# thetengda/OKVIS2-X

Measured on AMD Instinct MI355X. Metric: Gauss-Newton iters/sec on 50-KF/2000-landmark window; ATE vs CPU ref, higher is better.
Workload: dtype f64; 1 GPU; 2048 independent S50 windows (50 KF / 2000 landmarks / 16000 reprojections, 49 IMU factors), DENSE_SCHUR + DOGLEG, all tolerances 0; windows_total=2048, windows_per_gpu=2048, parallelism=replicas x1 (one window batch per GPU, no collective in the loop)

## Files before the change

include/okvisgpu.h:

```cpp
#ifndef OKVISGPU_H_
#define OKVISGPU_H_

#include <stdint.h>

#ifdef __cplusplus
extern "C" {
#endif

#define OKVISGPU_ABI_VERSION 6

typedef enum okvisgpu_status {
  OKVISGPU_OK = 0,
  OKVISGPU_ERR_INVALID_ARGUMENT = 1,
  OKVISGPU_ERR_UNSUPPORTED = 2,
  OKVISGPU_ERR_DEVICE = 3,
  OKVISGPU_ERR_OUT_OF_MEMORY = 4,
  OKVISGPU_ERR_NO_PROBLEM = 5,
  OKVISGPU_ERR_NUMERICAL = 6
} okvisgpu_status;

typedef enum okvisgpu_distortion {
  OKVISGPU_DIST_NONE = 0,
  OKVISGPU_DIST_RADTAN = 1,
  OKVISGPU_DIST_EQUIDISTANT = 2,
// ... 225 lines not shown
  const double* sample_gyr_acc;
} okvisgpu_imu_append_batch;
int okvisgpu_imu_append(okvisgpu_ctx* ctx, const okvisgpu_imu_append_batch* batch, int32_t* steps);

typedef struct okvisgpu_graph okvisgpu_graph;
int okvisgpu_graph_load(const char* path, const okvisgpu_camera* cameras, int32_t n_cameras,
                        const okvisgpu_imu_params* imu, okvisgpu_graph** out);
const okvisgpu_problem* okvisgpu_graph_problem(okvisgpu_graph* g);
int okvisgpu_graph_ids(const okvisgpu_graph* g, uint64_t* state_ids, int64_t* state_t_ns, uint64_t* landmark_ids);
void okvisgpu_graph_destroy(okvisgpu_graph* g);
int okvisgpu_graph_save(const okvisgpu_problem* p, const int64_t* state_t_ns, const char* path);

typedef struct okvisgpu_problem_stats {
  int32_t n_windows;
  int32_t cholesky_launches;
  int64_t n_poses, n_speed_biases, n_landmarks, n_landmarks_free, n_extrinsics_free;
  int64_t n_observations, n_visits, n_imu, n_imu_samples, n_pose_priors, n_sb_priors, n_relpose;
  int64_t reduced_dim;
  int64_t s_tiles_nonzero;
  int64_t s_tiles_dense;
  int64_t n_block_pairs, n_visit_segments, n_partial_blocks;
  int64_t arena_bytes;
  int64_t cholesky_split_windows;
} okvisgpu_problem_stats;
int okvisgpu_get_stats(okvisgpu_ctx* ctx, okvisgpu_problem_stats* stats);

int okvisgpu_plan_window(const okvisgpu_problem* problem, int32_t nested_dissection, int64_t* info,
                         uint8_t* tile_nz, int32_t* step_launch, int32_t* natural);

int okvisgpu_get_params(okvisgpu_ctx* ctx);

int okvisgpu_evaluate(okvisgpu_ctx* ctx, int32_t window, double* cost);

int okvisgpu_linearize_reduce(okvisgpu_ctx* ctx, int32_t window, int32_t jacobi_scaling, double mu,
                              double* S, double* rhs, double* cost, int32_t* dim_out);

int okvisgpu_eval_reprojection(okvisgpu_ctx* ctx, int32_t window, double* r, double* J_pose,
                               double* J_landmark);
int okvisgpu_eval_imu(okvisgpu_ctx* ctx, int32_t window, int32_t redo_always, double* r, double* J);
int okvisgpu_eval_relpose(okvisgpu_ctx* ctx, int32_t window, double* r, double* J);
int okvisgpu_eval_host(okvisgpu_ctx* ctx, int32_t window, double* r, double* J);

typedef struct okvisgpu_synth_config {
  int32_t n_keyframes;
  int32_t n_landmarks;
  int32_t n_observations;
// ... 31 lines not shown
```

okvis2-x_amd/csrc/chol_tiles.hpp:

```cpp
#pragma once
#include "dev_clock.hpp"
#include "device_problem.hpp"
#include "okvisgpu_math.hpp"

namespace okg {

constexpr int kLd = kTile + 1;


typedef double dbl4 __attribute__((ext_vector_type(4)));

__device__ __forceinline__ bool cholSelect(const DevProblem& P, int w) {
  const WinState& s = P.st[w];
  return !s.done && s.need_gn && !s.gn_failed;
}

__device__ __forceinline__ int tileBlocks(const DevProblem& P, int w, int k) {
  const int fdim = P.win_fdim[w], g0 = P.win_sgap[2 * w], gl = P.win_sgap[2 * w + 1];
  int end = min(fdim - kTile * k, kTile);
  if (gl > 0 && g0 >= kTile * k && g0 < kTile * (k + 1)) end = min(end, g0 - kTile * k);
  return max(1, (end + 15) >> 4);
}

struct TileSrc {
// ... 297 lines not shown
__host__ __device__ constexpr bool persistentCaller(int kCaller) { return kCaller >= 10; }
template <int kCaller>
__device__ __forceinline__ void xStoreRows16(const double* sX, double* Li, int q, int g, int lane) {
  double2 v[3];
#pragma unroll
  for (int it = 0; it < 3; ++it) {
    const int e = min(64 * g + lane + 192 * it, 511), r = 16 * q + (e >> 5), c = 2 * (e & 31);
    v[it] = double2{(c <= r) ? sX[r * kLd + c] : 0.0, (c + 1 <= r) ? sX[r * kLd + c + 1] : 0.0};
  }
#pragma unroll
  for (int it = 0; it < 3; ++it) {
    const int e = 64 * g + lane + 192 * it, r = 16 * q + (e >> 5), c = 2 * (e & 31);
    if (e < 512 && (!persistentCaller(kCaller) || c <= r)) *gmemw(reinterpret_cast<double2*>(Li + r * kTile + c)) = v[it];
  }
}

__host__ __device__ constexpr bool teamCaller(int kCaller) { return kCaller >= 20; }
constexpr int kPotrfBarriers = 3;
template <int kCaller>
__device__ __forceinline__ void potrfSync(int* sFl, int& tgen, int lane) {
  if (teamCaller(kCaller)) waveBarrier<true>(&sFl[4], tgen, 4, lane);
  else ldsBarrier();
}
template <int kCaller>
__device__ __forceinline__ bool potrfTileBody(const double* Sg, int64_t ld, double* Li, double* workk, double* sA, double* sX,
                                              double* sy, double* sRl, int* sFl, int t, bool haveTile, int tgen0, int nq) {
  const int wave = t >> 6, lane = t & 63;
  int tgen = tgen0;
  CLK_INIT
  if (!haveTile) loadTile(Sg, ld, 0, 0, sA, t);
  nq = __builtin_amdgcn_readfirstlane(nq);
#pragma unroll
  for (int u = 0; u < 16; ++u) {
    const int e = t + 256 * u;
    sX[(e >> 6) * kLd + (e & 63)] = 0.0;
  }
  if (t < 4) sFl[t] = 0;
  potrfSync<kCaller>(sFl, tgen, lane);
  CLK(4)
  if (wave == 0) {
    const int i = lane;
    if (i >= 16 * nq) {
      sX[i * kLd + i] = 1.0;
      sy[kTile + i] = sy[i];
    }
    double xp[8];
#pragma unroll
    for (int k = 0; k < 8; ++k) xp[k] = 0.0;
#pragma unroll 1
    for (int s = 0; s < 2 * nq; ++s) {
      const int c0 = 8 * s;
      CLK(25)
      if (s >= 2 && !waitFlag<true>(&sFl[1], s - 1, &sFl[2])) break;
      CLK(21)
      double r[8], x[8], rl[8];
#pragma unroll
      for (int k = 0; k < 8; ++k) r[k] = sA[i * kLd + c0 + k];
      if (s >= 1) {
#pragma unroll
        for (int hb = 0; hb < 2; ++hb) {
          double Lq[4][8];
#pragma unroll
          for (int c = 0; c < 4; ++c)
// ... 44 lines not shown
      if (s & 1) {
        const int q = s >> 1;
        if (g == 0) xDiag16(sA, sX, q, lane);
        waveBarrier<true>(&sFl[3], gen, 3, lane);
        if (g < q) xOffDiag16(sA, sX, q, g, lane);
        waveBarrier<true>(&sFl[3], gen, 3, lane);
        if (g == 0) yBlock16(sX, sy, q, lane);
        for (int qs = q, qe = q + 1 < nq ? q + 1 : 4; qs < qe; ++qs) xStoreRows16<kCaller>(sX, Li, qs, g, lane);
      }
    }
  }
  potrfSync<kCaller>(sFl, tgen, lane);
  CLK(5)
  if (sFl[2]) return false;
  if (t < kTile) {
    const double y = sy[kTile + t];
    sy[t] = y;
    if (!persistentCaller(kCaller)) gmemw(workk)[t] = y;
  }
  potrfSync<kCaller>(sFl, tgen, lane);
  CLK(10)
  return true;
}
template <int kCaller>
__device__ __noinline__ bool potrfTile(const double* Sg, int64_t ld, double* Li, double* workk, double* sA, double* sX, double* sy,
                                      double* sRl, int* sFl, int t, bool haveTile, int tgen0 = 0, int nq = 4) {
  return potrfTileBody<kCaller>(Sg, ld, Li, workk, sA, sX, sy, sRl, sFl, t, haveTile, tgen0, nq);
}

__device__ __forceinline__ void accToLds(double* s, const dbl4 acc[2][2], int t) {
  const int wave = t >> 6, lane = t & 63;
  const int r0 = 32 * (wave >> 1), c0 = 32 * (wave & 1);
#pragma unroll
  for (int a = 0; a < 2; ++a)
#pragma unroll
    for (int b = 0; b < 2; ++b)
#pragma unroll
      for (int reg = 0; reg < 4; ++reg) s[(r0 + 16 * a + (lane >> 4) + 4 * reg) * kLd + c0 + 16 * b + (lane & 15)] = acc[a][b][reg];
}
__device__ __forceinline__ void accSubToLds(double* s, const dbl4 c[2][2], const dbl4 acc[2][2], int t) {
  const int wave = t >> 6, lane = t & 63;
  const int r0 = 32 * (wave >> 1), c0 = 32 * (wave & 1);
#pragma unroll
  for (int a = 0; a < 2; ++a)
#pragma unroll
    for (int b = 0; b < 2; ++b)
#pragma unroll
      for (int reg = 0; reg < 4; ++reg)
        s[(r0 + 16 * a + (lane >> 4) + 4 * reg) * kLd + c0 + 16 * b + (lane & 15)] = c[a][b][reg] - acc[a][b][reg];
}
// ... 82 lines not shown
__device__ __forceinline__ void panelRhsVector(const double* sX, const double* sy, double* sz, double* sP, int t,
                                               Sync sync = Sync()) {
  const int c = t & 63, q = t >> 6;
  double a = 0.0;
#pragma unroll
  for (int r = 16 * q; r < 16 * q + 16; ++r) a += (r >= c) ? sX[r * kLd + c] * sy[r] : 0.0;
  sP[q * kTile + c] = a;
  sync();
  if (t < kTile) sz[t] = (sP[t] + sP[kTile + t]) + (sP[2 * kTile + t] + sP[3 * kTile + t]);
  sync();
}

__device__ __forceinline__ double panelRhsRow(const double* sA, const double* sz, int t) {
  const int row = t >> 2, q = t & 3;
  double a = 0.0;
#pragma unroll
  for (int c = 16 * q; c < 16 * q + 16; ++c) a += sA[row * kLd + c] * sz[c];
  a += __shfl_xor(a, 1, 64);
  a += __shfl_xor(a, 2, 64);
  return a;
}

template <class Sync = WgSync>
__device__ __forceinline__ void panelTile(const double* Aik, double* Lik, int64_t ld, double* worki, double* sA, const double* sX, const double* sz,
                          int t, double* defer = nullptr, Sync sync = Sync()) {
  loadTile(Aik, ld, 0, 0, sA, t);
  sync();
  dbl4 acc[4];
  mfmaPanelRows(sA, sX, acc, t);
  {
    const int row = t >> 2, q = t & 3;
    const double a = panelRhsRow(sA, sz, t);
    if (q == 0) {
      if (defer) defer[row] = a;
      else worki[row] -= a;
    }
  }
  sync();
  storePanelRows(Lik, ld, acc, t);
}


constexpr int kBsThreads = 1024;
constexpr int kBsPre = 3;
struct BsOps {
  double2 v[kBsPre][2];
  double2 li[2];
};
template <bool UPPER>
__device__ __forceinline__ const double* bsTile(const double* S, int64_t ld, int I, int i) {
  return UPPER ? S + (int64_t)I * kTile * ld + i * kTile : S + (int64_t)i * kTile * ld + I * kTile;
}
template <bool UPPER>
__device__ __forceinline__ void bsLoad(const double* S, int64_t ld, const double* Linv, const int* lst, int I, int vt,
                                       BsOps& o) {
  const int c2 = 2 * (vt & 31), rg = vt >> 5;
#ifdef OKG_BS_DUMMY_DIAG
  const int dummy = I;
#else
  const int dummy = lst[0] > 0 ? lst[1] : I;
#endif
#pragma unroll
// ... 116 lines not shown
```

okvis2-x_amd/csrc/device_problem.hpp:

```cpp
#pragma once

#include <cstdint>

namespace okg {

constexpr int kCamDoubles = 13;
constexpr int kTile = 64;
constexpr int16_t kNoUpdate = 32767;
constexpr int kImuLin = 15 + 15 * 30;
constexpr int kImuState = 526;
constexpr int kHostIn = 40;
constexpr int kHostOut = 1 + kImuLin;

constexpr int kObsLin = 8;
constexpr int kSegHG = 28;
constexpr int kSegUz = 8;
constexpr int kLmGroupVisits = 256;
__host__ __device__ constexpr bool fewWindows(int nWin, int cuCount) { return 4 * nWin <= cuCount; }
constexpr int kLmGroupMax = 64;
constexpr int kLmPartStage = 2048;
constexpr int kAsmLightMax = 24;
constexpr int kManyWindows = 64;
constexpr int kLmgInfo = 8;
constexpr int kImuHess = 465 + 30;
constexpr int kGrpRed = 8;
constexpr int kVisitZ = 18;

enum ContribType : int32_t {
  C_VISIT = 0,
  C_PAIR = 1,
  C_IMU = 2,
// ... 188 lines not shown
  int32_t n_asm_ppl;
  const int32_t* pair_win;
  const int32_t* pair_fi;
  const int32_t* pair_fj;
  const int32_t* pair_cbegin;
  const int32_t* pair_runs;
  const Contrib* pair_contrib;

  double* S;
  double* W;
  double* Linv;
  const int64_t* win_linvoff;
  const int32_t* tile_items;
  const int32_t* chol_root_items;
  int32_t n_chol_roots;
  int32_t n_chol_launches;
  const int32_t* chol_upd_items;
  const int32_t* chol_upd_begin;
  const int32_t* h_upd_begin;
  int32_t chol_schedule;
  const uint8_t* tile_nz;
  const int16_t* tile_fu;
  const int64_t* win_tnzoff;
  int32_t n_tiles;
  double* chol_defer;
  const int64_t* win_defoff;
  double* fwdF;
  const int64_t* win_fwdoff;
  double* sF;   double* sL;
  double* diagF; double* diagL;
  double* hdF;
  double* gF;   double* gL;
  double* rhsF;
  double* yF;   double* yL;
  double* gnF;  double* gnL;
  double* dgF;  double* dgL;
  double* vF;   double* vL;
  double* stepF; double* stepL;

  WinState* st;
  DevOptions opt;
};

constexpr int kTwoPoseOut = 6 + 36 + 7 + 36 + 6;
struct TwoPoseDev {
  int32_t n_edges, n_cam;
// ... 17 lines not shown
```

okvis2-x_amd/csrc/kernels_chol.hip:

```cpp
#include "chol_tiles.hpp"
#include "launch.hpp"

namespace okg {

#ifndef OKG_CHOL_OCC
#define OKG_CHOL_OCC 2
#endif

template <int MODE>
__global__ __launch_bounds__(256, OKG_CHOL_OCC) void k_cholesky(const DevProblem* __restrict__ Pp) {
  const DevProblem& P = *Pp;
  const int w = MODE == 1 ? (int)(blockIdx.x >> 1) : (int)blockIdx.x, part = MODE == 1 ? (int)(blockIdx.x & 1) : 0;
  if (!cholSelect(P, w)) return;
  const int64_t ld = P.win_fpad[w];
  const int T = (int)(ld / kTile);
  const int tL = MODE == 0 ? 0 : P.win_bsplit[2 * w], tS = MODE == 0 ? 0 : P.win_bsplit[2 * w + 1];
  const bool split = MODE != 0 && tS > 0;
  if ((MODE == 1 && part == 1 && !split) || (MODE == 2 && !split)) return;
  const int k0 = !split ? 0 : (MODE == 2 ? tS : (part == 0 ? 0 : tL));
  const int k1 = !split ? T : (MODE == 2 ? T : (part == 0 ? tL : tS));
  const int jEnd = split && MODE == 1 && part == 1 ? tS : T;
  const bool finish = !split || MODE == 2;
  const TileSrc cur = tileSrc(P, w, ld);
  double* W = P.W + P.win_soff[w];
  double* Linv = P.Linv + P.win_linvoff[w];
  const uint8_t* nz = P.tile_nz + P.win_tnzoff[w];
  double* work = P.fwdF + P.win_fwdoff[w];
  double* defer = split ? P.chol_defer + P.win_defoff[w] : nullptr;
  __shared__ double sA[kTile * kLd];
// ... 53 lines not shown
          }
        } else {
          dbl4 c[2][2], acc[2][2];
          loadC(cur.at(i, j, k), ld, c, t);
          mfmaTileNT(aBuf, bBuf, acc, t);
          storeTileSub(Cij, ld, c, acc, t);
        }
        ldsBarrier();
      }
    }
    return inLds;
  };
  if (MODE == 2) {
    for (int k = tL; k < tS; ++k) {
      for (int i = tS; i < T; ++i)
        if (nz[i * T + k] && t < kTile)
          sxDyn[i * kTile + t] -= defer[((size_t)(i - tS) * (tS - tL) + (k - tL)) * kTile + t];
      __syncthreads();
      bandUpdate(k, tS, false);
      __syncthreads();
    }
  }
  bool haveDiag = false;
  for (int k = k0; k < k1; ++k) {
    CLK(11)
    if (t < kTile) sy[t] = sxDyn[k * kTile + t];
    __syncthreads();
    if (!potrfTile<10 + MODE>(cur.at(k, k, k), ld, Linv + (int64_t)k * kTile * kTile, nullptr, sA, sX,
                   sy, sRl, sFl, t, haveDiag, 0, tileBlocks(P, w, k))) {
      if (t == 0) P.st[w].gn_failed = 1;
      return;
    }
    if (t < kTile) sxDyn[k * kTile + t] = sy[t];
    CLK(0)
    tStep = t;
    asm volatile("" : "+v"(tStep));
    panelRhsVector(sX, sy, sy + kTile, sA, t);
    for (int i = k + 1; i < T; ++i)
      if (nz[i * T + k])
        panelTile(cur.at(i, k, k), W + i * kTile * ld + k * kTile, ld, sxDyn + i * kTile, sA, sX, sy + kTile, tStep,
                  i >= jEnd ? defer + ((size_t)(i - tS) * (tS - tL) + (k - tL)) * kTile : nullptr);
    __syncthreads();
    CLK(1)
    haveDiag = bandUpdate(k, 0, true);
  }
  CLK(2)
// ... 223 lines not shown
```

okvis2-x_amd/csrc/runtime.cpp:

```cpp
#include <hip/hip_runtime.h>

#include <algorithm>
#include <array>
#include <cfloat>
#include <chrono>
#include <climits>
#include <cmath>
#include <condition_variable>
#include <cstdio>
#include <cstdlib>
#include <cstring>
#include <functional>
#include <map>
#include <memory>
#include <mutex>
#include <numeric>
#include <stdexcept>
#include <string>
#include <thread>
#include <vector>

#include "../../include/okvisgpu.h"
#include "device_problem.hpp"
#include "launch.hpp"
// ... 91 lines not shown
  std::vector<int32_t> fb_win, fb_kind, fb_index, fb_off, fb_cbegin;
  std::vector<int32_t> win_sgap, f_nat, win_fnat, win_bsplit;
  std::vector<int64_t> win_defoff;
  int64_t defer_total = 0;
  bool any_split = false;
  bool nd = false;
  int lmg_visits = kLmGroupVisits, lmg_lms = kLmGroupMax;
  std::vector<int32_t> chol_root_items;
  int n_chol_launches = 1;
  std::vector<Contrib> fb_contrib;
  std::vector<int32_t> pair_win, pair_fi, pair_fj, pair_cbegin, pair_runs;
  std::vector<int32_t> asm_pp_items, asm_sb_items, asm_ppl_items;
  std::vector<int32_t> chol_upd_items, chol_upd_begin, tile_items;
  int64_t n_panels = 0;
  int64_t n_band_updates = 0;
  int64_t n_band_updates_diag = 0;
  std::vector<Contrib> pair_contrib;
  int64_t s_total = 0, linv_total = 0, fwd_total = 0;
  std::vector<std::vector<uint8_t>> tileNz;
  std::vector<uint8_t> tile_nz;
  std::vector<std::vector<int16_t>> tileFu;
  std::vector<int16_t> tile_fu;
  std::vector<int64_t> win_tnzoff;
  std::vector<int> tileT;
  int f_total = 0;
  int max_fpad = 0;
  int max_panels = 0;
};

template <class T>
void appendN(std::vector<T>& v, const T* src, size_t n) {
  if (n) v.insert(v.end(), src, src + n);
}

bool lossValid(const okvisgpu_loss& L) {
  switch (L.kind) {
    case OKVISGPU_LOSS_NONE: return true;
    case OKVISGPU_LOSS_TOLERANT: return L.a >= 0.0 && L.b > 0.0 && std::isfinite(L.a) && std::isfinite(L.b);
    case OKVISGPU_LOSS_CAUCHY: case OKVISGPU_LOSS_TUKEY: case OKVISGPU_LOSS_HUBER: case OKVISGPU_LOSS_SOFTLONE:
    case OKVISGPU_LOSS_ARCTAN: return L.a > 0.0 && std::isfinite(L.a);
  }
  return false;
}

void lossRho(const okvisgpu_loss& L, double s, double* rho) {
  const double a = L.a;
// ... 168 lines not shown
    }
  }
}

#ifdef OKG_ANALYSE_TIMING
double g_atime[16];
std::chrono::steady_clock::time_point g_alast;
#define ATIME(i)                                                                                    \
  {                                                                                                 \
    const auto now = std::chrono::steady_clock::now();                                             \
    g_atime[i] += std::chrono::duration<double, std::milli>(now - g_alast).count();                 \
    g_alast = now;                                                                                  \
  }
#else
#define ATIME(i)
#endif

void symbolicFill(std::vector<uint8_t>& nz, int T) {
  for (int k = 0; k < T; ++k)
    for (int i = k + 1; i < T; ++i)
      if (nz[(size_t)i * T + k])
        for (int j = k + 1; j <= i; ++j)
          if (nz[(size_t)j * T + k]) nz[(size_t)i * T + j] = 1;
}
int cholSchedule(const std::vector<uint8_t>& nz, int T, std::vector<int>& L, std::vector<int>& last) {
  L.assign(T, 0);
  last.assign((size_t)T * T, -1);
  int n = 1;
  for (int k = 0; k < T; ++k) {
    int lk = std::max(1, last[(size_t)k * T + k] + 1);
    bool any = false;
    for (int i = k + 1; i < T; ++i)
      if (nz[(size_t)i * T + k])
        for (int j = k + 1; j <= i; ++j)
          if (nz[(size_t)j * T + k]) {
            lk = std::max(lk, last[(size_t)i * T + j] + 1);
            any = true;
          }
    L[k] = lk;
    if (!any) continue;
    for (int i = k + 1; i < T; ++i)
      if (nz[(size_t)i * T + k])
        for (int j = k + 1; j <= i; ++j)
          if (nz[(size_t)j * T + k]) last[(size_t)i * T + j] = lk;
    n = std::max(n, lk + 1);
  }
// ... 812 lines not shown
    }
    auto interleave = [&](std::vector<std::vector<int32_t>>& qq, int perWG, std::vector<int32_t>& out) {
      std::vector<size_t> pos(nq, 0);
      bool more = true;
      while (more) {
        more = false;
        for (int x = 0; x < nq; ++x)
          for (int i = 0; i < perWG; ++i) {
            const bool has = pos[x] < qq[x].size();
            out.push_back(has ? qq[x][pos[x]++] : -1);
          }
        for (int x = 0; x < nq; ++x) more = more || pos[x] < qq[x].size();
      }
      while (!out.empty() && out.back() < 0) out.pop_back();
    };
    interleave(q, 4, B.asm_pp_items);
    interleave(ql, 16, B.asm_ppl_items);
  }
  for (int w = 0; w < B.n_win; ++w) {
    B.win_tnzoff.push_back((int64_t)B.tile_nz.size());
    B.tile_nz.insert(B.tile_nz.end(), B.tileNz[w].begin(), B.tileNz[w].end());
    B.tile_fu.insert(B.tile_fu.end(), B.tileFu[w].begin(), B.tileFu[w].end());
    const int T = B.tileT[w];
    for (int k = 0; k < T; ++k) {
      int np = 0;
      for (int i = k + 1; i < T; ++i) np += B.tileNz[w][(size_t)i * T + k] ? 1 : 0;
      B.max_panels = std::max(B.max_panels, np);
    }
  }
  for (int w = 0; w < B.n_win; ++w) {
    const int T = B.tileT[w];
    for (int i = 0; i < T; ++i)
      for (int j = 0; j <= i; ++j)
        if (B.tileNz[w][(size_t)i * T + j]) { B.tile_items.push_back(w); B.tile_items.push_back(i); B.tile_items.push_back(j); }
  }
  B.lm_visit_begin.push_back((int)B.visit_pose.size());
  B.lmg_begin.push_back((int)B.lm_win.size());
  {
    B.win_lmg_range.assign(2 * (size_t)B.n_win, 0);
    const int ng = (int)B.lmg_begin.size() - 1;
    std::vector<int> first(B.n_win, -1), last(B.n_win, -1);
    for (int g = 0; g < ng; ++g) {
      const int w = B.lm_win[B.lmg_begin[g]];
      if (first[w] < 0) first[w] = g;
      last[w] = g;
    }
// ... 523 lines not shown
    const size_t o_sbp_block = upl(B.sbp_block), o_sbp_win = upl(B.sbp_win), o_sbp_meas = upl(B.sbp_meas),
                 o_sbp_L = upl(B.sbp_L);
    const size_t o_sbp_lin0 = scratch(sizeof(double) * 90 * D.n_sbprior),
                 o_sbp_lin1 = scratch(sizeof(double) * 90 * D.n_sbprior),
                 o_sbp_cost0 = scratch(sizeof(double) * D.n_sbprior), o_sbp_cost1 = scratch(sizeof(double) * D.n_sbprior),
                 o_sbp_jv = scratch(sizeof(double) * 3 * D.n_sbprior);
    const size_t o_rp_blocks = upl(B.rp_blocks), o_rp_win = upl(B.rp_win), o_rp_flags = upl(B.rp_flags),
                 o_rp_kind = upl(B.rp_kind),
                 o_rp_dx = upl(B.rp_dx), o_rp_J = upl(B.rp_J), o_rp_lp = upl(B.rp_lp);
    const size_t o_rp_lin0 = scratch(sizeof(double) * kRelPoseLin * D.n_relpose),
                 o_rp_lin1 = scratch(sizeof(double) * kRelPoseLin * D.n_relpose),
                 o_rp_cost0 = scratch(sizeof(double) * D.n_relpose), o_rp_cost1 = scratch(sizeof(double) * D.n_relpose),
                 o_rp_jv = scratch(sizeof(double) * 3 * D.n_relpose), o_wrpr = upl(B.win_rp_range);
    const size_t o_wfoff = upl(B.win_foff), o_wfdim = upl(B.win_fdim), o_wfpad = upl(B.win_fpad),
                 o_wsoff = upl(B.win_soff), o_wlinv = upl(B.win_linvoff), o_wfwd = upl(B.win_fwdoff), o_wpr = upl(B.win_pose_range), o_wsr = upl(B.win_sb_range),
                 o_wlr = upl(B.win_lm_range), o_wlgr = upl(B.win_lmg_range), o_wor = upl(B.win_obs_range), o_wir = upl(B.win_imu_range),
                 o_wppr = upl(B.win_pp_range), o_wsbpr = upl(B.win_sbp_range);
    const size_t o_fbw = upl(B.fb_win), o_fbk = upl(B.fb_kind), o_fbi = upl(B.fb_index), o_fbo = upl(B.fb_off),
                 o_fbcb = upl(B.fb_cbegin), o_fbc = upl(B.fb_contrib);
    const size_t o_pw = upl(B.pair_win), o_pfi = upl(B.pair_fi), o_pfj = upl(B.pair_fj), o_pcb = upl(B.pair_cbegin),
                 o_pc = upl(B.pair_contrib);
    const size_t o_pruns = upl(B.pair_runs);
    const size_t o_tnz = upl(B.tile_nz), o_tnzoff = upl(B.win_tnzoff), o_tfu = upl(B.tile_fu);
    const size_t o_app = upl(B.asm_pp_items), o_asb = upl(B.asm_sb_items), o_appl = upl(B.asm_ppl_items);
    const size_t o_ti = upl(B.tile_items);
    const size_t o_cri = upl(B.chol_root_items), o_cui = upl(B.chol_upd_items), o_cub = upl(B.chol_upd_begin);
    const size_t o_wsgap = upl(B.win_sgap), o_wbsp = upl(B.win_bsplit), o_wdef = upl(B.win_defoff);
    const size_t nf = std::max(1, B.f_total), nl3 = std::max<size_t>(1, (size_t)3 * D.n_lm);
    const size_t o_S = scratch(sizeof(double) * std::max<int64_t>(1, B.s_total));
    const size_t o_W = scratch(sizeof(double) * std::max<int64_t>(1, B.s_total));
    const size_t o_Linv = scratch(sizeof(double) * std::max<int64_t>(1, B.linv_total));
    const size_t o_fwd = scratch(sizeof(double) * std::max<int64_t>(1, B.fwd_total));
    const size_t o_defer = scratch(sizeof(double) * std::max<int64_t>(1, B.defer_total));
    size_t of[10], ol[7];
    for (int i = 0; i < 10; ++i) of[i] = scratch(sizeof(double) * nf);
    for (int i = 0; i < 7; ++i) ol[i] = scratch(sizeof(double) * nl3);
    const size_t o_st = scratch(sizeof(WinState) * D.n_win);
    const size_t o_self = scratch(sizeof(DevProblem));
    const size_t upSize = (A.size + 255) & ~size_t(255);
    const size_t total = upSize + AS.size;
    if (!arena || total > arenaCap) {
      if (arena) {
        HIPCHK(hipFree(arena));
        arena = nullptr;
        arenaCap = 0;
      }
// ... 58 lines not shown
    D.pp_block = ip(o_pp_block); D.pp_win = ip(o_pp_win); D.pp_meas = dp(o_pp_meas); D.pp_L = dp(o_pp_L);
    D.pp_lin[0] = dp(o_pp_lin0); D.pp_lin[1] = dp(o_pp_lin1); D.pp_cost[0] = dp(o_pp_cost0);
    D.pp_cost[1] = dp(o_pp_cost1); D.pp_jv = dp(o_pp_jv);
    D.sbp_block = ip(o_sbp_block); D.sbp_win = ip(o_sbp_win); D.sbp_meas = dp(o_sbp_meas); D.sbp_L = dp(o_sbp_L);
    D.sbp_lin[0] = dp(o_sbp_lin0); D.sbp_lin[1] = dp(o_sbp_lin1); D.sbp_cost[0] = dp(o_sbp_cost0);
    D.sbp_cost[1] = dp(o_sbp_cost1); D.sbp_jv = dp(o_sbp_jv);
    D.win_foff = ip(o_wfoff); D.win_fdim = ip(o_wfdim); D.win_fpad = ip(o_wfpad); D.win_soff = lp(o_wsoff);
    D.win_pose_range = ip(o_wpr); D.win_sb_range = ip(o_wsr); D.win_lm_range = ip(o_wlr); D.win_lmg_range = ip(o_wlgr);
    D.win_obs_range = ip(o_wor); D.win_imu_range = ip(o_wir); D.win_pp_range = ip(o_wppr);
    D.win_sbp_range = ip(o_wsbpr);
    D.win_rp_range = ip(o_wrpr);
    D.rp_blocks = ip(o_rp_blocks); D.rp_win = ip(o_rp_win); D.rp_flags = up(o_rp_flags); D.rp_kind = up(o_rp_kind);
    D.rp_dx = dp(o_rp_dx); D.rp_J = dp(o_rp_J); D.rp_lp = dp(o_rp_lp);
    D.rp_lin[0] = dp(o_rp_lin0); D.rp_lin[1] = dp(o_rp_lin1);
    D.rp_cost[0] = dp(o_rp_cost0); D.rp_cost[1] = dp(o_rp_cost1); D.rp_jv = dp(o_rp_jv);
    D.fb_win = ip(o_fbw); D.fb_kind = ip(o_fbk); D.fb_index = ip(o_fbi); D.fb_off = ip(o_fbo);
    D.fb_cbegin = ip(o_fbcb); D.fb_contrib = reinterpret_cast<const Contrib*>(base + place(o_fbc));
    D.pair_win = ip(o_pw); D.pair_fi = ip(o_pfi); D.pair_fj = ip(o_pfj); D.pair_cbegin = ip(o_pcb);
    D.pair_contrib = reinterpret_cast<const Contrib*>(base + place(o_pc));
    D.pair_runs = ip(o_pruns);
    D.tile_nz = reinterpret_cast<const uint8_t*>(base + place(o_tnz));
    D.tile_fu = reinterpret_cast<const int16_t*>(base + place(o_tfu));
    D.win_tnzoff = reinterpret_cast<const int64_t*>(base + place(o_tnzoff));
    D.chol_root_items = ip(o_cri);
    D.n_chol_roots = (int)B.chol_root_items.size() / 3;
    D.n_chol_launches = B.n_chol_launches;
    D.chol_upd_items = ip(o_cui); D.chol_upd_begin = ip(o_cub);
    D.h_upd_begin = B.chol_upd_begin.data();
    D.win_sgap = ip(o_wsgap);
    D.win_bsplit = ip(o_wbsp);
    D.chol_schedule = 1;
    D.asm_pp_items = ip(o_app); D.asm_sb_items = ip(o_asb);
    D.n_asm_pp = (int)B.asm_pp_items.size(); D.n_asm_sb = (int)B.asm_sb_items.size();
    D.asm_ppl_items = ip(o_appl); D.n_asm_ppl = (int)B.asm_ppl_items.size();
    D.tile_items = ip(o_ti);
    D.n_tiles = (int)(B.tile_items.size() / 3);
    D.S = dp(o_S);
    D.W = dp(o_W);
    D.Linv = dp(o_Linv);
    D.win_linvoff = lp(o_wlinv);
    D.fwdF = dp(o_fwd);
    D.chol_defer = dp(o_defer);
    D.win_defoff = lp(o_wdef);
    D.win_fwdoff = lp(o_wfwd);
    double** fv[10] = {&D.sF, &D.diagF, &D.hdF, &D.gF, &D.rhsF, &D.yF, &D.gnF, &D.dgF, &D.vF, &D.stepF};
    for (int i = 0; i < 10; ++i) *fv[i] = dp(of[i]);
// ... 670 lines not shown
  for (int w = 0; w < B.n_win; ++w) {
    const okvisgpu_problem* p = B.probs[w];
    for (int c = 0; c < p->n_cameras; ++c) st->n_extrinsics_free += B.pose_f[B.pose_base[w] + p->n_poses + c] >= 0;
  }
  for (uint8_t f : B.lm_free) st->n_landmarks_free += f != 0;
  st->n_observations = P.n_obs;
  st->n_visits = P.n_visit;
  st->n_imu = P.n_imu;
  st->n_imu_samples = (int64_t)B.imu_ts.size();
  st->n_pose_priors = P.n_pprior;
  st->n_sb_priors = P.n_sbprior;
  st->n_relpose = P.n_relpose;
  st->cholesky_launches = B.n_chol_launches;
  st->reduced_dim = 0;
  for (int d : B.win_fnat) st->reduced_dim += d;
  st->s_tiles_nonzero = (int64_t)B.tile_items.size() / 3;
  for (int T : B.tileT) st->s_tiles_dense += (int64_t)T * (T + 1) / 2;
  st->n_block_pairs = P.n_pair;
  st->n_visit_segments = P.n_seg;
  st->n_partial_blocks = P.n_part;
  st->arena_bytes = (int64_t)c->arenaBytes;
  st->cholesky_split_windows = 0;
  for (size_t w = 0; w + 1 < c->B.win_bsplit.size(); w += 2) st->cholesky_split_windows += c->B.win_bsplit[w + 1] > 0;
  return OKVISGPU_OK;
}

int okvisgpu_plan_window(const okvisgpu_problem* p, int32_t nested_dissection, int64_t* info, uint8_t* tile_nz,
                         int32_t* step_launch, int32_t* natural) {
  if (!p) return OKVISGPU_ERR_INVALID_ARGUMENT;
  try {
    HostBatch B;
    B.nd = nested_dissection != 0;
#ifdef OKG_ANALYSE_TIMING
    for (double& x : g_atime) x = 0.0;
    g_alast = std::chrono::steady_clock::now();
#endif
    analyse({p}, {}, B);
#ifdef OKG_ANALYSE_TIMING
    std::fprintf(stderr, "analyse ms:");
    for (int i = 0; i < 11; ++i) std::fprintf(stderr, " [%d] %.3f", i, g_atime[i]);
    std::fprintf(stderr, "\n");
#endif
    const int T = B.tileT[0], fpad = B.win_fpad[0];
    const auto& nz = B.tileNz[0];
    std::vector<int> L, last;
    const int nl = cholSchedule(nz, T, L, last);
// ... 353 lines not shown
```

okvis2-x_amd/okvisgpu/__init__.py:

```python
from __future__ import annotations

import ctypes as C
import os
from typing import Optional

import numpy as np

_HERE = os.path.dirname(os.path.abspath(__file__))
PKG_ROOT = os.path.dirname(_HERE)
REPO_ROOT = os.path.dirname(PKG_ROOT)
LIB_PATH = os.environ.get("OKVISGPU_LIB") or os.path.join(PKG_ROOT, "libokvisgpu.so")

IMU_STATE_DOUBLES = 526

DIST_NONE, DIST_RADTAN, DIST_EQUIDISTANT, DIST_RADTAN8 = 0, 1, 2, 3
DENSE_SCHUR, SPARSE_NORMAL_CHOLESKY = 0, 1
TERMINATION = {0: "CONVERGENCE", 1: "NO_CONVERGENCE", 2: "FAILURE", 3: "USER_SUCCESS"}

_dp = C.POINTER(C.c_double)
_ip = C.POINTER(C.c_int32)
_lp = C.POINTER(C.c_int64)
_up = C.POINTER(C.c_uint8)


# ... 112 lines not shown
                ("residual_evaluation_time_s", C.c_double), ("jacobian_evaluation_time_s", C.c_double),
                ("step_time_s", C.c_double)]

    def as_dict(self):
        d = {k: getattr(self, k) for k, _ in self._fields_}
        d["termination"] = TERMINATION.get(self.termination_type, "?")
        return d


class SynthConfig(C.Structure):
    _fields_ = [("n_keyframes", C.c_int32), ("n_landmarks", C.c_int32), ("n_observations", C.c_int32),
                ("max_obs_per_landmark", C.c_int32), ("kf_dt_s", C.c_double), ("imu_rate_hz", C.c_double),
                ("pixel_noise", C.c_double), ("init_sigma_pos", C.c_double), ("init_sigma_rot", C.c_double),
                ("init_sigma_lm", C.c_double), ("init_sigma_vel", C.c_double), ("seed", C.c_uint64),
                ("n_relpose", C.c_int32), ("relpose_stride", C.c_int32), ("relpose_kind", C.c_int32),
                ("do_extrinsics", C.c_int32), ("extrinsics_sigma_r", C.c_double), ("extrinsics_sigma_alpha", C.c_double)]


class ProblemStats(C.Structure):
    _fields_ = [("n_windows", C.c_int32), ("cholesky_launches", C.c_int32)] + [(k, C.c_int64) for k in (
        "n_poses", "n_speed_biases", "n_landmarks", "n_landmarks_free", "n_extrinsics_free", "n_observations",
        "n_visits", "n_imu", "n_imu_samples", "n_pose_priors", "n_sb_priors", "n_relpose", "reduced_dim",
        "s_tiles_nonzero", "s_tiles_dense", "n_block_pairs", "n_visit_segments", "n_partial_blocks",
        "arena_bytes", "cholesky_split_windows")]

    def as_dict(self):
        return {k: getattr(self, k) for k, _ in self._fields_}


class ImuAppendBatch(C.Structure):
    _fields_ = [("n", C.c_int32), ("imu_params", ImuParams), ("state", _dp), ("t1_old_ns", _lp), ("t1_new_ns", _lp),
                ("speed_biases", _dp), ("sample_begin", _ip), ("sample_t_ns", _lp), ("sample_gyr_acc", _dp)]


class TwoPoseEdges(C.Structure):
    _fields_ = [("n_edges", C.c_int32), ("ref_pose", _dp), ("other_pose", _dp),
                ("n_cameras", C.c_int32), ("cameras", C.POINTER(Camera)), ("extrinsics", _dp),
                ("landmark_begin", _ip), ("landmarks", _dp), ("obs_begin", _ip), ("obs_other", _up),
                ("obs_camera", _ip), ("obs_keypoint", _dp), ("obs_sqrt_info", _dp), ("obs_cauchy", _up)]


EXPORTED_SYMBOLS = [
    "okvisgpu_abi_version", "okvisgpu_default_options", "okvisgpu_device_count", "okvisgpu_ctx_create",
    "okvisgpu_ctx_destroy", "okvisgpu_last_error", "okvisgpu_set_problems", "okvisgpu_update_params",
    "okvisgpu_set_block_constant", "okvisgpu_solve", "okvisgpu_get_params", "okvisgpu_evaluate",
    "okvisgpu_linearize_reduce", "okvisgpu_eval_reprojection", "okvisgpu_eval_imu",
    "okvisgpu_synth_default_config", "okvisgpu_synth_create", "okvisgpu_synth_problem",
# ... 472 lines not shown
```

Baseline: 205,300 window-iterations/s.

## Carry Cholesky trailing-update tiles in registers across steps with wave role split

```diff
diff --git a/include/okvisgpu.h b/include/okvisgpu.h
--- a/include/okvisgpu.h
+++ b/include/okvisgpu.h
@@ -271,6 +271,7 @@
   int64_t n_block_pairs, n_visit_segments, n_partial_blocks;
   int64_t arena_bytes;
   int64_t cholesky_split_windows;
+  int64_t cholesky_tiles_carried, cholesky_tiles_roundtrip;
 } okvisgpu_problem_stats;
 int okvisgpu_get_stats(okvisgpu_ctx* ctx, okvisgpu_problem_stats* stats);
 
diff --git a/okvis2-x_amd/csrc/chol_tiles.hpp b/okvis2-x_amd/csrc/chol_tiles.hpp
--- a/okvis2-x_amd/csrc/chol_tiles.hpp
+++ b/okvis2-x_amd/csrc/chol_tiles.hpp
@@ -343,7 +343,7 @@
   if (teamCaller(kCaller)) waveBarrier<true>(&sFl[4], tgen, 4, lane);
   else ldsBarrier();
 }
-template <int kCaller>
+template <int kCaller, int kRole = -1>
 __device__ __forceinline__ bool potrfTileBody(const double* Sg, int64_t ld, double* Li, double* workk, double* sA, double* sX,
                                               double* sy, double* sRl, int* sFl, int t, bool haveTile, int tgen0, int nq) {
   const int wave = t >> 6, lane = t & 63;
@@ -359,7 +359,7 @@
   if (t < 4) sFl[t] = 0;
   potrfSync<kCaller>(sFl, tgen, lane);
   CLK(4)
-  if (wave == 0) {
+  if (kRole == 0 || (kRole < 0 && wave == 0)) {
     const int i = lane;
     if (i >= 16 * nq) {
       sX[i * kLd + i] = 1.0;
@@ -450,10 +450,10 @@
   CLK(10)
   return true;
 }
-template <int kCaller>
+template <int kCaller, int kRole = -1>
 __device__ __noinline__ bool potrfTile(const double* Sg, int64_t ld, double* Li, double* workk, double* sA, double* sX, double* sy,
                                       double* sRl, int* sFl, int t, bool haveTile, int tgen0 = 0, int nq = 4) {
-  return potrfTileBody<kCaller>(Sg, ld, Li, workk, sA, sX, sy, sRl, sFl, t, haveTile, tgen0, nq);
+  return potrfTileBody<kCaller, kRole>(Sg, ld, Li, workk, sA, sX, sy, sRl, sFl, t, haveTile, tgen0, nq);
 }
 
 __device__ __forceinline__ void accToLds(double* s, const dbl4 acc[2][2], int t) {
@@ -582,11 +582,9 @@
 }
 
 template <class Sync = WgSync>
-__device__ __forceinline__ void panelTile(const double* Aik, double* Lik, int64_t ld, double* worki, double* sA, const double* sX, const double* sz,
-                          int t, double* defer = nullptr, Sync sync = Sync()) {
-  loadTile(Aik, ld, 0, 0, sA, t);
+__device__ __forceinline__ void panelTileStaged(double* Lik, int64_t ld, double* worki, double* sA, const double* sX, const double* sz,
+                                                int t, dbl4 acc[4], double* defer = nullptr, Sync sync = Sync()) {
   sync();
-  dbl4 acc[4];
   mfmaPanelRows(sA, sX, acc, t);
   {
     const int row = t >> 2, q = t & 3;
@@ -598,6 +596,195 @@
   }
   sync();
   storePanelRows(Lik, ld, acc, t);
+}
+template <class Sync = WgSync>
+__device__ __forceinline__ void panelTile(const double* Aik, double* Lik, int64_t ld, double* worki, double* sA, const double* sX, const double* sz,
+                          int t, double* defer = nullptr, Sync sync = Sync()) {
+  loadTile(Aik, ld, 0, 0, sA, t);
+  dbl4 acc[4];
+  panelTileStaged(Lik, ld, worki, sA, sX, sz, t, acc, defer, sync);
+}
+
+constexpr int kCarryF4 = kCarrySlotD ? 2 : 0;
+struct CarryF {
+  dbl4 b[6];
+};
+struct CarryD {
+  dbl4 b[4];
+};
+__device__ __forceinline__ int carryFH(int g) { return g < kCarryF4 ? g : g - 1; }
+__device__ __forceinline__ int carryFRb(int g, int e) { return g != kCarryF4 ? 2 * carryFH(g) + e / 3 : e; }
+__device__ __forceinline__ int carryFCb(int g, int e) { return g != kCarryF4 ? e % 3 : 3; }
+__device__ __forceinline__ int64_t carryFAt(int g, int e, int reg, int lane, int64_t ld) {
+  return (int64_t)(16 * carryFRb(g, e) + (lane >> 4) + 4 * reg) * ld + 16 * carryFCb(g, e) + (lane & 15);
+}
+#define OKG_ARM(tag) asm volatile("; carry arm " tag)
+template <int N>
+__device__ __forceinline__ void carryFLoadN(const double* A, int64_t ld, CarryF& s, int g, int lane) {
+#pragma unroll
+  for (int e = 0; e < N; ++e)
+#pragma unroll
+    for (int reg = 0; reg < 4; ++reg) s.b[e][reg] = gmem(A)[carryFAt(g, e, reg, lane, ld)];
+}
+template <int N>
+__device__ __forceinline__ void carryFStoreN(double* A, int64_t ld, const CarryF& s, int g, int lane) {
+#pragma unroll
+  for (int e = 0; e < N; ++e)
+#pragma unroll
+    for (int reg = 0; reg < 4; ++reg) gmemw(A)[carryFAt(g, e, reg, lane, ld)] = s.b[e][reg];
+}
+template <int N>
+__device__ __forceinline__ void carryFToLdsN(double* sT, const CarryF& s, int g, int lane) {
+#pragma unroll
+  for (int e = 0; e < N; ++e)
+#pragma unroll
+    for (int reg = 0; reg < 4; ++reg) sT[carryFAt(g, e, reg, lane, kLd)] = s.b[e][reg];
+}
+__device__ __forceinline__ void carryFLoad(const double* A, int64_t ld, CarryF& s, int g, int lane) {
+  if (g != kCarryF4) {
+    carryFLoadN<6>(A, ld, s, g, lane);
+    OKG_ARM("carryFLoad6");
+  } else {
+    carryFLoadN<4>(A, ld, s, g, lane);
+    OKG_ARM("carryFLoad4");
+  }
+}
+__device__ __forceinline__ void carryFStore(double* A, int64_t ld, const CarryF& s, int g, int lane) {
+  if (g != kCarryF4) {
+    carryFStoreN<6>(A, ld, s, g, lane);
+    OKG_ARM("carryFStore6");
+  } else {
+    carryFStoreN<4>(A, ld, s, g, lane);
+    OKG_ARM("carryFStore4");
+  }
+}
+__device__ __forceinline__ void carryFToLds(double* sT, const CarryF& s, int g, int lane) {
+  if (g != kCarryF4) {
+    carryFToLdsN<6>(sT, s, g, lane);
+    OKG_ARM("carryFToLds6");
+  } else {
+    carryFToLdsN<4>(sT, s, g, lane);
+    OKG_ARM("carryFToLds4");
+  }
+}
+__device__ __forceinline__ void carryFMfmaSub(const double* sA, const double* sB, CarryF& s, int g, int lane) {
+  const int lr = lane & 15, lk = lane >> 4;
+  dbl4 acc[6];
+#pragma unroll
+  for (int e = 0; e < 6; ++e) acc[e] = dbl4{0.0, 0.0, 0.0, 0.0};
+  if (g != kCarryF4) {
+    const double* pa = sA + (32 * carryFH(g) + lr) * kLd + lk;
+    const double* pb = sB + lr * kLd + lk;
+#pragma unroll 4
+    for (int kk = 0; kk < kTile; kk += 4) {
+      double av[2], bv[3];
+#pragma unroll
+      for (int a = 0; a < 2; ++a) av[a] = pa[16 * a * kLd + kk];
+#pragma unroll
+      for (int b = 0; b < 3; ++b) bv[b] = pb[16 * b * kLd + kk];
+#pragma unroll
+      for (int a = 0; a < 2; ++a)
+#pragma unroll
+        for (int b = 0; b < 3; ++b)
+          acc[3 * a + b] = __builtin_amdgcn_mfma_f64_16x16x4f64(av[a], bv[b], acc[3 * a + b], 0, 0, 0);
+    }
+#pragma unroll
+    for (int e = 0; e < 6; ++e) s.b[e] = s.b[e] - acc[e];
+    OKG_ARM("carryFMfmaSub6");
+  } else {
+    const double* pa = sA + lr * kLd + lk;
+    const double* pb = sB + (48 + lr) * kLd + lk;
+#pragma unroll 4
+    for (int kk = 0; kk < kTile; kk += 4) {
+      const double bv = pb[kk];
+#pragma unroll
+      for (int a = 0; a < 4; ++a) acc[a] = __builtin_amdgcn_mfma_f64_16x16x4f64(pa[16 * a * kLd + kk], bv, acc[a], 0, 0, 0);
+    }
+#pragma unroll
+    for (int e = 0; e < 4; ++e) s.b[e] = s.b[e] - acc[e];
+    OKG_ARM("carryFMfmaSub4");
+  }
+}
+__device__ __forceinline__ int carryDRb(int g, int e) { return g == 2 ? 3 : (g == 1 ? 2 : (e == 0 ? 0 : 1)); }
+__device__ __forceinline__ int carryDCb(int g, int e) { return g > 0 ? e : (e == 2 ? 1 : 0); }
+__device__ __forceinline__ int64_t carryDAt(int g, int e, int reg, int lane, int64_t ld) {
+  return (int64_t)(16 * carryDRb(g, e) + (lane >> 4) + 4 * reg) * ld + 16 * carryDCb(g, e) + (lane & 15);
+}
+template <int N>
+__device__ __forceinline__ void carryDLoadN(const double* A, int64_t ld, CarryD& s, int g, int lane) {
+#pragma unroll
+  for (int e = 0; e < N; ++e)
+#pragma unroll
+    for (int reg = 0; reg < 4; ++reg) s.b[e][reg] = gmem(A)[carryDAt(g, e, reg, lane, ld)];
+}
+template <int N>
+__device__ __forceinline__ void carryDStoreN(double* A, int64_t ld, const CarryD& s, int g, int lane) {
+#pragma unroll
+  for (int e = 0; e < N; ++e)
+#pragma unroll
+    for (int reg = 0; reg < 4; ++reg) gmemw(A)[carryDAt(g, e, reg, lane, ld)] = s.b[e][reg];
+}
+template <int N>
+__device__ __forceinline__ void carryDToLdsN(double* sT, const CarryD& s, int g, int lane) {
+#pragma unroll
+  for (int e = 0; e < N; ++e)
+#pragma unroll
+    for (int reg = 0; reg < 4; ++reg) sT[carryDAt(g, e, reg, lane, kLd)] = s.b[e][reg];
+}
+template <int N>
+__device__ __forceinline__ void carryDMfmaSubN(const double* sL, CarryD& s, int g, int lane) {
+  const int lr = lane & 15, lk = lane >> 4;
+  int ra[N], rb[N];
+  dbl4 acc[N];
+#pragma unroll
+  for (int e = 0; e < N; ++e) {
+    ra[e] = (16 * carryDRb(g, e) + lr) * kLd + lk;
+    rb[e] = (16 * carryDCb(g, e) + lr) * kLd + lk;
+    acc[e] = dbl4{0.0, 0.0, 0.0, 0.0};
+  }
+#pragma unroll 4
+  for (int kk = 0; kk < kTile; kk += 4) {
+#pragma unroll
+    for (int e = 0; e < N; ++e) acc[e] = __builtin_amdgcn_mfma_f64_16x16x4f64(sL[ra[e] + kk], sL[rb[e] + kk], acc[e], 0, 0, 0);
+  }
+#pragma unroll
+  for (int e = 0; e < N; ++e) s.b[e] = s.b[e] - acc[e];
+}
+__device__ __forceinline__ void carryDLoad(const double* A, int64_t ld, CarryD& s, int g, int lane) {
+  if (g == 2) {
+    carryDLoadN<4>(A, ld, s, g, lane);
+    OKG_ARM("carryDLoad4");
+  } else {
+    carryDLoadN<3>(A, ld, s, g, lane);
+    OKG_ARM("carryDLoad3");
+  }
+}
+__device__ __forceinline__ void carryDStore(double* A, int64_t ld, const CarryD& s, int g, int lane) {
+  if (g == 2) {
+    carryDStoreN<4>(A, ld, s, g, lane);
+    OKG_ARM("carryDStore4");
+  } else {
+    carryDStoreN<3>(A, ld, s, g, lane);
+    OKG_ARM("carryDStore3");
+  }
+}
+__device__ __forceinline__ void carryDToLds(double* sT, const CarryD& s, int g, int lane) {
+  if (g == 2) {
+    carryDToLdsN<4>(sT, s, g, lane);
+    OKG_ARM("carryDToLds4");
+  } else {
+    carryDToLdsN<3>(sT, s, g, lane);
+    OKG_ARM("carryDToLds3");
+  }
+}
+__device__ __forceinline__ void carryDMfmaSub(const double* sL, CarryD& s, int g, int lane) {
+  if (g == 2) {
+    carryDMfmaSubN<4>(sL, s, g, lane);
+    OKG_ARM("carryDMfmaSub4");
+  } else {
+    carryDMfmaSubN<3>(sL, s, g, lane);
+    OKG_ARM("carryDMfmaSub3");
+  }
 }
 
 
diff --git a/okvis2-x_amd/csrc/device_problem.hpp b/okvis2-x_amd/csrc/device_problem.hpp
--- a/okvis2-x_amd/csrc/device_problem.hpp
+++ b/okvis2-x_amd/csrc/device_problem.hpp
@@ -7,6 +7,13 @@
 constexpr int kCamDoubles = 13;
 constexpr int kTile = 64;
 constexpr int16_t kNoUpdate = 32767;
+#ifndef OKG_CHOL_CARRY_D
+#define OKG_CHOL_CARRY_D 0
+#endif
+constexpr bool kCarrySlotD = OKG_CHOL_CARRY_D != 0;
+constexpr int kCarryRec = 8;
+constexpr int kCarryNone = 255;
+constexpr int kCarryFromSlot = 1, kCarryToW = 2;
 constexpr int kImuLin = 15 + 15 * 30;
 constexpr int kImuState = 526;
 constexpr int kHostIn = 40;
@@ -241,6 +248,7 @@
   const uint8_t* tile_nz;
   const int16_t* tile_fu;
   const int64_t* win_tnzoff;
+  const uint8_t* chol_carry;
   int32_t n_tiles;
   double* chol_defer;
   const int64_t* win_defoff;
diff --git a/okvis2-x_amd/csrc/kernels_chol.hip b/okvis2-x_amd/csrc/kernels_chol.hip
--- a/okvis2-x_amd/csrc/kernels_chol.hip
+++ b/okvis2-x_amd/csrc/kernels_chol.hip
@@ -1,3 +1,5 @@
+#include <type_traits>
+
 #include "chol_tiles.hpp"
 #include "launch.hpp"
 
@@ -5,6 +7,9 @@
 
 #ifndef OKG_CHOL_OCC
 #define OKG_CHOL_OCC 2
+#endif
+#ifndef OKG_CHOL_CARRY
+#define OKG_CHOL_CARRY 1
 #endif
 
 template <int MODE>
@@ -104,6 +109,163 @@
     }
   }
   bool haveDiag = false;
+#if OKG_CHOL_CARRY
+  if constexpr (MODE == 0) {
+    const uint8_t* plan = P.chol_carry + (P.win_linvoff[w] >> 9);
+    auto carrySteps = [&](auto roleTag) -> bool {
+      constexpr int ROLE = decltype(roleTag)::value;
+      CarryF slotF;
+      CarryD slotD;
+      if constexpr (ROLE == 1) {
+#pragma unroll
+        for (int e = 0; e < 6; ++e) slotF.b[e] = dbl4{0.0, 0.0, 0.0, 0.0};
+#pragma unroll
+        for (int e = 0; e < 4; ++e) slotD.b[e] = dbl4{0.0, 0.0, 0.0, 0.0};
+      }
+      bool haveDiag = false;
+      for (int k = 0; k < T; ++k) {
+        CLK(11)
+        int ts = t;
+        asm volatile("" : "+v"(ts));
+        CarryD dNext;
+        if (ts < kTile) sy[ts] = sxDyn[k * kTile + ts];
+        __syncthreads();
+        bool ok;
+        if constexpr (ROLE == 0)
+          ok = potrfTile<10, 0>(cur.at(k, k, k), ld, Linv + (int64_t)k * kTile * kTile, nullptr, sA, sX, sy, sRl, sFl, ts,
+                                haveDiag, 0, tileBlocks(P, w, k));
+        else
+          ok = potrfTileBody<10, 1>(cur.at(k, k, k), ld, Linv + (int64_t)k * kTile * kTile, nullptr, sA, sX, sy, sRl, sFl,
+                                    ts, haveDiag, 0, tileBlocks(P, w, k));
+        if (!ok) {
+          if (ts == 0) P.st[w].gn_failed = 1;
+          return false;
+        }
+        if (ts < kTile) sxDyn[k * kTile + ts] = sy[ts];
+        CLK(0)
+        const int lane = ts & 63, g = __builtin_amdgcn_readfirstlane(ts >> 6) - 1;
+        const uint2 pr = *gmem(reinterpret_cast<const uint2*>(plan + kCarryRec * k));
+        const unsigned p0 = __builtin_amdgcn_readfirstlane(pr.x), p1 = __builtin_amdgcn_readfirstlane(pr.y);
+        const int fPanel = p0 & 0xff, fI = (p0 >> 8) & 0xff, fJ = (p0 >> 16) & 0xff;
+        const bool fFromSlot = (p0 >> 24) & kCarryFromSlot, fToW = (p0 >> 24) & kCarryToW;
+        const int dHeld = p1 & 0xff, dNew = (p1 >> 16) & 0xff;
+        const bool dToW = (p1 >> 8) & kCarryToW;
+        panelRhsVector(sX, sy, sy + kTile, sA, ts);
+        int jFirst = -1, iLast = -1;
+        for (int i = k + 1; i < T; ++i)
+          if (nz[i * T + k]) {
+            if (jFirst < 0) jFirst = i;
+            iLast = i;
+          }
+        dbl4 lFirst[4];
+        for (int i = k + 1; i < T; ++i) {
+          if (!nz[i * T + k]) continue;
+          double* Lik = W + i * kTile * ld + k * kTile;
+          if (i == fPanel) {
+            if constexpr (ROLE == 1) carryFToLds(sA, slotF, g, lane);
+          } else {
+            loadTile(cur.at(i, k, k), ld, 0, 0, sA, ts);
+          }
+          dbl4 acc[4];
+          panelTileStaged(Lik, ld, sxDyn + i * kTile, sA, sX, sy + kTile, ts, acc);
+          if (i == iLast) {
+            panelRowsToLds(sA, acc, ts);
+          } else if (i == jFirst) {
+#pragma unroll
+            for (int cb = 0; cb < 4; ++cb) lFirst[cb] = acc[cb];
+          }
+        }
+        const bool twoHeld = jFirst >= 0 && jFirst != iLast;
+        if (twoHeld) panelRowsToLds(sX, lFirst, ts);
+        ldsBarrier();
+        CLK(1)
+        int xHeld = twoHeld ? jFirst : -1;
+        bool reads = false, wFresh = true;
+        haveDiag = false;
+        for (int i = T - 1; i > k; --i) {
+          if (!nz[i * T + k]) continue;
+          const bool aInX = xHeld == i;
+          const double* aBuf = aInX ? sX : sA;
+          bool aLoaded = aInX || i == iLast;
+          for (int j = k + 1; j <= i; ++j) {
+            if (!nz[j * T + k]) continue;
+            const bool stages = !aLoaded || (j != i && (aInX || xHeld != j));
+            if (stages) {
+              if (wFresh) __syncthreads();
+              else if (reads) ldsBarrier();
+              wFresh = reads = false;
+            }
+            int tu = ts;
+            asm volatile("" : "+v"(tu));
+            const int lane = tu & 63;
+            if (!aLoaded) {
+              loadTile(W + i * kTile * ld + k * kTile, ld, 0, 0, sA, tu);
+              aLoaded = true;
+            }
+            const double* bBuf = aBuf;
+            if (j != i) {
+              if (aInX) {
+                loadTile(W + j * kTile * ld + k * kTile, ld, 0, 0, sA, tu);
+                bBuf = sA;
+              } else {
+                if (xHeld != j) loadTile(W + j * kTile * ld + k * kTile, ld, 0, 0, sX, tu);
+                xHeld = j;
+                bBuf = sX;
+              }
+            }
+            if (stages) ldsBarrier();
+            reads = true;
+            double* Cij = W + i * kTile * ld + j * kTile;
+            if (kCarrySlotD && j == i && i == dHeld) {
+              if constexpr (ROLE == 1) carryDMfmaSub(aBuf, slotD, g, lane);
+              if (i == k + 1) {
+                ldsBarrier();
+                if constexpr (ROLE == 1) carryDToLds(sA, slotD, g, lane);
+                haveDiag = true;
+              } else if (dToW) {
+                if constexpr (ROLE == 1) carryDStore(Cij, ld, slotD, g, lane);
+              }
+            } else if (kCarrySlotD && j == i && i == dNew) {
+              if constexpr (ROLE == 1) {
+                carryDLoad(cur.at(i, j, k), ld, dNext, g, lane);
+                carryDMfmaSub(aBuf, dNext, g, lane);
+              }
+            } else if (j != i && i == fI && j == fJ) {
+              if constexpr (ROLE == 1) {
+                if (!fFromSlot) carryFLoad(cur.at(i, j, k), ld, slotF, g, lane);
+                carryFMfmaSub(aBuf, bBuf, slotF, g, lane);
+                if (fToW) carryFStore(Cij, ld, slotF, g, lane);
+              }
+            } else if (j == i) {
+              dbl4 c[3], acc[3];
+              loadCDiag(cur.at(i, j, k), ld, c, tu);
+              mfmaDiagNT(aBuf, acc, tu);
+              if (i == k + 1) {
+                ldsBarrier();
+                diagSubToLds(sA, c, acc, tu);
+                haveDiag = true;
+              } else {
+                storeDiagSub(Cij, ld, c, acc, tu);
+              }
+            } else {
+              dbl4 c[2][2], acc[2][2];
+              loadC(cur.at(i, j, k), ld, c, tu);
+              mfmaTileNT(aBuf, bBuf, acc, tu);
+              storeTileSub(Cij, ld, c, acc, tu);
+            }
+          }
+        }
+        if constexpr (ROLE == 1) {
+          if (kCarrySlotD && dNew != kCarryNone) slotD = dNext;
+        }
+      }
+      return true;
+    };
+    const bool chain = __builtin_amdgcn_readfirstlane(t >> 6) == 0;
+    const bool ok = chain ? carrySteps(std::integral_constant<int, 0>()) : carrySteps(std::integral_constant<int, 1>());
+    if (!ok) return;
+  } else
+#endif
   for (int k = k0; k < k1; ++k) {
     CLK(11)
     if (t < kTile) sy[t] = sxDyn[k * kTile + t];
diff --git a/okvis2-x_amd/csrc/runtime.cpp b/okvis2-x_amd/csrc/runtime.cpp
--- a/okvis2-x_amd/csrc/runtime.cpp
+++ b/okvis2-x_amd/csrc/runtime.cpp
@@ -137,6 +137,8 @@
   std::vector<std::vector<int16_t>> tileFu;
   std::vector<int16_t> tile_fu;
   std::vector<int64_t> win_tnzoff;
+  std::vector<uint8_t> chol_carry;
+  int64_t n_carried = 0, n_roundtrip = 0;
   std::vector<int> tileT;
   int f_total = 0;
   int max_fpad = 0;
@@ -351,6 +353,78 @@
       if (nz[(size_t)i * T + k])
         for (int j = k + 1; j <= i; ++j)
           if (nz[(size_t)j * T + k]) nz[(size_t)i * T + j] = 1;
+}
+void carryPlan(const std::vector<uint8_t>& nz, int T, std::vector<uint8_t>& plan, int64_t& carried, int64_t& roundtrip) {
+  const size_t base = plan.size();
+  plan.resize(base + (size_t)kCarryRec * T, (uint8_t)kCarryNone);
+  const bool on = T < kCarryNone;
+  auto at = [&](int i, int j) { return nz[(size_t)i * T + j] != 0; };
+  auto target = [&](int i, int j, int k) { return k < j && j <= i && j < T && at(i, k) && at(j, k); };
+  int fi = -1, fj = -1, di = -1;
+  for (int k = 0; k < T; ++k) {
+    uint8_t* r = plan.data() + base + (size_t)kCarryRec * k;
+    r[3] = r[5] = r[7] = 0;
+    bool fFree = true;
+    if (fi >= 0 && fj == k) {
+      r[0] = (uint8_t)fi;
+      fi = -1;
+    }
+    if (fi >= 0) {
+      fFree = false;
+      r[1] = (uint8_t)fi;
+      r[2] = (uint8_t)fj;
+      r[3] = kCarryFromSlot;
+      if (fj == k + 1 || target(fi, fj, k + 1)) {
+        ++carried;
+      } else {
+        r[3] |= kCarryToW;
+        ++roundtrip;
+        fi = -1;
+      }
+    }
+    bool dFree = true;
+    if (di >= 0) {
+      r[4] = (uint8_t)di;
+      r[5] = kCarryFromSlot;
+      if (di == k + 1) {
+        di = -1;
+      } else if (target(di, di, k + 1)) {
+        dFree = false;
+        ++carried;
+      } else {
+        r[5] |= kCarryToW;
+        ++roundtrip;
+        di = -1;
+      }
+    }
+    for (int i = k + 1; i < T; ++i) {
+      if (!at(i, k)) continue;
+      for (int j = k + 1; j <= i; ++j) {
+        if (!at(j, k)) continue;
+        if (i == j) {
+          if ((on && i == r[4]) || i == k + 1) continue;
+          if (on && kCarrySlotD && dFree && r[6] == kCarryNone && target(i, i, k + 1)) {
+            r[6] = (uint8_t)i;
+            ++carried;
+          } else {
+            ++roundtrip;
+          }
+        } else {
+          if (on && i == r[1] && j == r[2]) continue;
+          if (on && fFree && fi < 0 && (j == k + 1 || target(i, j, k + 1))) {
+            r[1] = (uint8_t)i;
+            r[2] = (uint8_t)j;
+            fi = i;
+            fj = j;
+            ++carried;
+          } else {
+            ++roundtrip;
+          }
+        }
+      }
+    }
+    if (r[6] != kCarryNone) di = r[6];
+  }
 }
 int cholSchedule(const std::vector<uint8_t>& nz, int T, std::vector<int>& L, std::vector<int>& last) {
   L.assign(T, 0);
@@ -1209,6 +1283,7 @@
     B.tile_nz.insert(B.tile_nz.end(), B.tileNz[w].begin(), B.tileNz[w].end());
     B.tile_fu.insert(B.tile_fu.end(), B.tileFu[w].begin(), B.tileFu[w].end());
     const int T = B.tileT[w];
+    carryPlan(B.tileNz[w], T, B.chol_carry, B.n_carried, B.n_roundtrip);
     for (int k = 0; k < T; ++k) {
       int np = 0;
       for (int i = k + 1; i < T; ++i) np += B.tileNz[w][(size_t)i * T + k] ? 1 : 0;
@@ -1778,6 +1853,7 @@
                  o_pc = upl(B.pair_contrib);
     const size_t o_pruns = upl(B.pair_runs);
     const size_t o_tnz = upl(B.tile_nz), o_tnzoff = upl(B.win_tnzoff), o_tfu = upl(B.tile_fu);
+    const size_t o_carry = upl(B.chol_carry);
     const size_t o_app = upl(B.asm_pp_items), o_asb = upl(B.asm_sb_items), o_appl = upl(B.asm_ppl_items);
     const size_t o_ti = upl(B.tile_items);
     const size_t o_cri = upl(B.chol_root_items), o_cui = upl(B.chol_upd_items), o_cub = upl(B.chol_upd_begin);
@@ -1882,6 +1958,7 @@
     D.tile_nz = reinterpret_cast<const uint8_t*>(base + place(o_tnz));
     D.tile_fu = reinterpret_cast<const int16_t*>(base + place(o_tfu));
     D.win_tnzoff = reinterpret_cast<const int64_t*>(base + place(o_tnzoff));
+    D.chol_carry = up(o_carry);
     D.chol_root_items = ip(o_cri);
     D.n_chol_roots = (int)B.chol_root_items.size() / 3;
     D.n_chol_launches = B.n_chol_launches;
@@ -2598,6 +2675,8 @@
   st->arena_bytes = (int64_t)c->arenaBytes;
   st->cholesky_split_windows = 0;
   for (size_t w = 0; w + 1 < c->B.win_bsplit.size(); w += 2) st->cholesky_split_windows += c->B.win_bsplit[w + 1] > 0;
+  st->cholesky_tiles_carried = B.n_carried;
+  st->cholesky_tiles_roundtrip = B.n_roundtrip;
   return OKVISGPU_OK;
 }
 
diff --git a/okvis2-x_amd/okvisgpu/__init__.py b/okvis2-x_amd/okvisgpu/__init__.py
--- a/okvis2-x_amd/okvisgpu/__init__.py
+++ b/okvis2-x_amd/okvisgpu/__init__.py
@@ -158,7 +158,7 @@
         "n_poses", "n_speed_biases", "n_landmarks", "n_landmarks_free", "n_extrinsics_free", "n_observations",
         "n_visits", "n_imu", "n_imu_samples", "n_pose_priors", "n_sb_priors", "n_relpose", "reduced_dim",
         "s_tiles_nonzero", "s_tiles_dense", "n_block_pairs", "n_visit_segments", "n_partial_blocks",
-        "arena_bytes", "cholesky_split_windows")]
+        "arena_bytes", "cholesky_split_windows", "cholesky_tiles_carried", "cholesky_tiles_roundtrip")]
 
     def as_dict(self):
         return {k: getattr(self, k) for k, _ in self._fields_}
```

Result: no change. 205,700 window-iterations/s, median of 6 (+0.2%).
